# shanice-l/UNOPose

Measured on AMD Instinct MI355X. Metric: (query,ref) pairs/sec forward, higher is better.
Workload: dtype bf16; 1 GPU; UNOPose.forward, batch 32 pairs/GPU, 2048 query pts, 5000->2048 reference pts, 196 coarse pts, 518x518 crops, DINOv2 ViT-B/14 reg4, random-init (trained-like) weights

## Files before the change

unopose_amd/csrc/attn.hip:

```cpp
#include "gemm_common.h"

namespace unopose {

template <int XOR>
__device__ __forceinline__ float swz_xor(float v) {
  constexpr int ctrl = XOR == 1 ? 0xB1 : XOR == 2 ? 0x4E : XOR == 4 ? 0x141 : 0x140;
  return __int_as_float(__builtin_amdgcn_update_dpp(0, __float_as_int(v), ctrl, 0xF, 0xF, false));
}
__device__ __forceinline__ float row16_max(float v) {
  v = fmaxf(v, swz_xor<1>(v));
  v = fmaxf(v, swz_xor<2>(v));
  v = fmaxf(v, swz_xor<4>(v));
  v = fmaxf(v, swz_xor<8>(v));
  return v;
}
__device__ __forceinline__ float row16_sum(float v) {
  v += swz_xor<1>(v);
  v += swz_xor<2>(v);
  v += swz_xor<4>(v);
  v += swz_xor<8>(v);
  return v;
}

__device__ __forceinline__ bf16x8 zero8() {
  bf16x8 z;
#pragma unroll
  for (int i = 0; i < 8; ++i) z[i] = (__bf16)0.f;
  return z;
}

constexpr int TA_NT = 14;
constexpr int TA_MP = TA_NT * 16;

template <bool RPE, int RW>
__global__ __launch_bounds__(256, 2) void token_attn_kernel(const u16 *__restrict__ q, int ldq,
                                                         const u16 *__restrict__ k, int ldk,
                                                         const u16 *__restrict__ vt, const u16 *__restrict__ qp,
                                                         int ldqp, const u16 *__restrict__ E, int n, int m,
                                                         float scale, u16 *__restrict__ out) {
  __shared__ __attribute__((aligned(16))) u16 Pl[4][16][TA_MP];
  __shared__ __attribute__((aligned(16))) u16 Al[RPE ? 4 : 1][8][64][8];
  const int b = blockIdx.y, lane = threadIdx.x & 63, wave = threadIdx.x >> 6;
  const int n0 = (blockIdx.x * 4 + wave) * RW;
  if (n0 >= n) return;
  const int li = lane & 15, kg = lane >> 4;
  const int a_nl = li >> 2, a_h = li & 3;
  const bool a_valid = a_nl < RW && n0 + a_nl < n;
  const u16 *Q = q + ((size_t)b * n + n0 + a_nl) * ldq;
  const u16 *K = k + (size_t)b * m * ldk;

  f32x4 acc[TA_NT];
#pragma unroll
  for (int t = 0; t < TA_NT; ++t) acc[t] = f32x4{0.f, 0.f, 0.f, 0.f};

  {
    bf16x8 qa[8];
#pragma unroll
    for (int ks = 0; ks < 8; ++ks) {
      const int kk = ks * 32 + kg * 8;
      qa[ks] = zero8();
      if (a_valid && (kk >> 6) == a_h) qa[ks] = *reinterpret_cast<const bf16x8 *>(Q + kk);
    }
    bf16x8 kb[2][TA_NT];
    auto load_k = [&](int ks, bf16x8 (&dst)[TA_NT]) {
#pragma unroll
      for (int t = 0; t < TA_NT; ++t) {
        const int mm = min(t * 16 + li, m - 1);
        dst[t] = *reinterpret_cast<const bf16x8 *>(K + (size_t)mm * ldk + ks * 32 + kg * 8);
      }
    };
    load_k(0, kb[0]);
#pragma unroll
    for (int ks = 0; ks < 8; ++ks) {
      if (ks + 1 < 8) load_k(ks + 1, kb[(ks + 1) & 1]);
#pragma unroll
      for (int t = 0; t < TA_NT; ++t) acc[t] = __builtin_amdgcn_mfma_f32_16x16x32_bf16(qa[ks], kb[ks & 1][t], acc[t], 0, 0, 0);
    }
  }
  if (RPE) {
    for (int nl = 0; nl < RW; ++nl) {
      if (n0 + nl >= n) break;
      const u16 *QP = qp + ((size_t)b * n + n0 + nl) * ldqp + a_h * 256;
      const u16 *En = E + ((size_t)b * n + n0 + nl) * (size_t)m * 256;
#pragma unroll
      for (int ks = 0; ks < 8; ++ks) {
        bf16x8 av = zero8();
        if (a_nl == nl) av = *reinterpret_cast<const bf16x8 *>(QP + ks * 32 + kg * 8);
        *reinterpret_cast<bf16x8 *>(&Al[wave][ks][lane][0]) = av;
      }
      const int nt_valid = (m + 15) >> 4;
      bf16x8 buf[3][8];
      auto load_tile = [&](int t, bf16x8 (&dst)[8]) {
        const u16 *Er = En + (size_t)min(t * 16 + li, m - 1) * 256 + kg * 8;
#pragma unroll
        for (int ks = 0; ks < 8; ++ks) dst[ks] = *reinterpret_cast<const bf16x8 *>(Er + ks * 32);
      };
      load_tile(0, buf[0]);
      if (1 < nt_valid) load_tile(1, buf[1]);
#pragma unroll
      for (int t = 0; t < TA_NT; ++t) {
        if (t >= nt_valid) continue;
        if (t + 2 < nt_valid) load_tile(t + 2, buf[(t + 2) % 3]);
#pragma unroll
        for (int ks = 0; ks < 8; ++ks) {
          const bf16x8 av = *reinterpret_cast<const bf16x8 *>(&Al[wave][ks][lane][0]);
          acc[t] = __builtin_amdgcn_mfma_f32_16x16x32_bf16(av, buf[t % 3][ks], acc[t], 0, 0, 0);
        }
      }
    }
  }
  float mx[4] = {-3e38f, -3e38f, -3e38f, -3e38f};
#pragma unroll
  for (int t = 0; t < TA_NT; ++t) {
    const bool ok = t * 16 + li < m;
#pragma unroll
    for (int h = 0; h < 4; ++h) {
      acc[t][h] = ok ? acc[t][h] * scale : -3e38f;
      mx[h] = fmaxf(mx[h], acc[t][h]);
    }
  }
  float sm[4];
#pragma unroll
  for (int h = 0; h < 4; ++h) {
    mx[h] = row16_max(mx[h]);
    sm[h] = 0.f;
  }
#pragma unroll
  for (int t = 0; t < TA_NT; ++t) {
    const bool ok = t * 16 + li < m;
#pragma unroll
    for (int h = 0; h < 4; ++h) {
      const float p = ok ? __expf(acc[t][h] - mx[h]) : 0.f;
      acc[t][h] = p;
      sm[h] += p;
    }
  }
#pragma unroll
  for (int h = 0; h < 4; ++h) sm[h] = 1.f / row16_sum(sm[h]);
#pragma unroll
  for (int t = 0; t < TA_NT; ++t)
#pragma unroll
    for (int h = 0; h < 4; ++h) Pl[wave][kg * 4 + h][t * 16 + li] = f2bf(acc[t][h] * sm[h]);
  __builtin_amdgcn_fence(__ATOMIC_RELEASE, "wavefront");
  __builtin_amdgcn_wave_barrier();
  __builtin_amdgcn_fence(__ATOMIC_ACQUIRE, "wavefront");
  bf16x8 pa[TA_MP / 32];
#pragma unroll
  for (int ks = 0; ks < TA_MP / 32; ++ks)
    pa[ks] = *reinterpret_cast<const bf16x8 *>(&Pl[wave][li][ks * 32 + kg * 8]);
  const u16 *VT = vt + (size_t)b * 256 * TA_MP;
  constexpr int PK = TA_MP / 32;
  bf16x8 vb[2][PK];
  auto load_v = [&](int nt, bf16x8 (&dst)[PK]) {
    const u16 *Vr = VT + (size_t)(nt * 16 + li) * TA_MP + kg * 8;
#pragma unroll
    for (int ks = 0; ks < PK; ++ks) dst[ks] = *reinterpret_cast<const bf16x8 *>(Vr + ks * 32);
  };
  load_v(0, vb[0]);
#pragma unroll
  for (int nt = 0; nt < 16; ++nt) {
    if (nt + 1 < 16) load_v(nt + 1, vb[(nt + 1) & 1]);
    f32x4 o = f32x4{0.f, 0.f, 0.f, 0.f};
#pragma unroll
    for (int ks = 0; ks < PK; ++ks) o = __builtin_amdgcn_mfma_f32_16x16x32_bf16(pa[ks], vb[nt & 1][ks], o, 0, 0, 0);
    if (kg < RW && n0 + kg < n) out[((size_t)b * n + n0 + kg) * 256 + nt * 16 + li] = f2bf(o[nt >> 2]);
  }
}

constexpr int TA_EPOL = 1;
constexpr int TA_RING = 2 * 8192;
constexpr int TA_ROWS = 4;

__global__ __launch_bounds__(256, 2) void token_attn_rpe_dma_kernel(const u16 *__restrict__ q, int ldq, const u16 *__restrict__ k, int ldk,
                                                                     const u16 *__restrict__ vt, const u16 *__restrict__ qp, int ldqp,
                                                                     const u16 *__restrict__ E, int n, int m, float scale, int B,
                                                                     u16 *__restrict__ out) {
  constexpr int RW = 4;
  __shared__ __attribute__((aligned(1024))) char ring[4][TA_RING];
  const int b = blockIdx.y, lane = threadIdx.x & 63, wave = __builtin_amdgcn_readfirstlane(threadIdx.x >> 6);
  const int li = lane & 15, kg = lane >> 4;
  const int a_nl = li >> 2, a_h = li & 3;
  const int nbase = (blockIdx.x * 4 + wave) * TA_ROWS;
#pragma unroll 1
  for (int n0 = nbase; n0 < min(n, nbase + TA_ROWS); n0 += RW) {
  const int rw_here = min(RW, min(n, nbase + TA_ROWS) - n0);
  const bool a_valid = a_nl < rw_here;
  const u16 *Q = q + ((size_t)b * n + n0 + a_nl) * ldq;
  const u16 *K = k + (size_t)b * m * ldk;

  f32x4 acc[TA_NT];
#pragma unroll
  for (int t = 0; t < TA_NT; ++t) acc[t] = f32x4{0.f, 0.f, 0.f, 0.f};
  const uint32_t lds0 = (uint32_t)(uintptr_t)(__attribute__((address_space(3))) char *)&ring[0][0] + (uint32_t)wave * TA_RING;
  const int nt_valid = (m + 15) >> 4;
  const int rows_w = rw_here;
  const int total = rows_w * nt_valid;
  const __amdgpu_buffer_rsrc_t e_rs = __builtin_amdgcn_make_buffer_rsrc((void *)E, 0, (int)min((size_t)B * n * m * 512, (size_t)0xFFFFFFFFu), 0x00020000);
  uint32_t voff[8];
#pragma unroll
  for (int j = 0; j < 8; ++j) {
    const int key = 2 * j + (lane >> 5);
    voff[j] = (uint32_t)(key * 512 + (((lane & 31) ^ key) << 4));
  }
  const uint32_t row0 = (uint32_t)(((size_t)b * n + n0) * (size_t)m * 512);
  auto issue_tile = [&](int s) {
    const int r = s / nt_valid, t = s - r * nt_valid;
    const uint32_t so = row0 + (uint32_t)r * (uint32_t)m * 512u + (uint32_t)t * 8192u;
    const uint32_t dst = lds0 + (uint32_t)(s & 1) * 8192u;
#pragma unroll
    for (int j = 0; j < 8; ++j) gemm_dma16<TA_EPOL>(dst + j * 1024, so + voff[j], e_rs, 0);
  };
  issue_tile(0);
  if (total > 1) issue_tile(1);
  bf16x8 myq[8];
  {
    const u16 *QP = qp + ((size_t)b * n + n0 + a_nl) * ldqp + a_h * 256;
#pragma unroll
    for (int ks = 0; ks < 8; ++ks) {
      myq[ks] = zero8();
      if (a_valid) myq[ks] = *reinterpret_cast<const bf16x8 *>(QP + ks * 32 + kg * 8);
    }
  }
  {
    bf16x8 qa[8];
#pragma unroll
    for (int ks = 0; ks < 8; ++ks) {
      const int kk = ks * 32 + kg * 8;
      qa[ks] = zero8();
      if (a_valid && (kk >> 6) == a_h) qa[ks] = *reinterpret_cast<const bf16x8 *>(Q + kk);
    }
    bf16x8 kb[2][TA_NT];
    auto load_k = [&](int ks, bf16x8 (&dst)[TA_NT]) {
#pragma unroll
      for (int t = 0; t < TA_NT; ++t) {
        const int mm = min(t * 16 + li, m - 1);
        dst[t] = *reinterpret_cast<const bf16x8 *>(K + (size_t)mm * ldk + ks * 32 + kg * 8);
      }
    };
    load_k(0, kb[0]);
#pragma unroll
    for (int ks = 0; ks < 8; ++ks) {
      if (ks + 1 < 8) load_k(ks + 1, kb[(ks + 1) & 1]);
#pragma unroll
      for (int t = 0; t < TA_NT; ++t) acc[t] = __builtin_amdgcn_mfma_f32_16x16x32_bf16(qa[ks], kb[ks & 1][t], acc[t], 0, 0, 0);
    }
  }
  const char *ringw = &ring[0][0] + wave * TA_RING;
  const uint32_t frag_off = (uint32_t)(li * 512);
  int s = 0;
  for (int nl = 0; nl < rows_w; ++nl) {
    bf16x8 av[8];
#pragma unroll
    for (int ks = 0; ks < 8; ++ks) av[ks] = a_nl == nl ? myq[ks] : zero8();
#pragma unroll
    for (int t = 0; t < TA_NT; ++t) {
      if (t >= nt_valid) continue;
      if (s + 1 < total)
        asm volatile("s_waitcnt vmcnt(8)" ::: "memory");
      else
        asm volatile("s_waitcnt vmcnt(0)" ::: "memory");
      __builtin_amdgcn_sched_barrier(0);
      const char *tb = ringw + (s & 1) * 8192;
      bf16x8 eb[8];
#pragma unroll
      for (int ks = 0; ks < 8; ++ks) eb[ks] = *reinterpret_cast<const bf16x8 *>(tb + frag_off + ((((ks << 2) | kg) ^ li) << 4));
      asm volatile("s_waitcnt lgkmcnt(0)" ::: "memory");
      __builtin_amdgcn_sched_barrier(0);
      if (s + 2 < total) issue_tile(s + 2);
#pragma unroll
      for (int ks = 0; ks < 8; ++ks) acc[t] = __builtin_amdgcn_mfma_f32_16x16x32_bf16(av[ks], eb[ks], acc[t], 0, 0, 0);
      ++s;
    }
  }
  float mx[4] = {-3e38f, -3e38f, -3e38f, -3e38f};
#pragma unroll
  for (int t = 0; t < TA_NT; ++t) {
    const bool ok = t * 16 + li < m;
#pragma unroll
    for (int h = 0; h < 4; ++h) {
      acc[t][h] = ok ? acc[t][h] * scale : -3e38f;
      mx[h] = fmaxf(mx[h], acc[t][h]);
    }
  }
  float sm[4];
#pragma unroll
  for (int h = 0; h < 4; ++h) {
    mx[h] = row16_max(mx[h]);
    sm[h] = 0.f;
  }
#pragma unroll
  for (int t = 0; t < TA_NT; ++t) {
    const bool ok = t * 16 + li < m;
#pragma unroll
    for (int h = 0; h < 4; ++h) {
      const float p = ok ? __expf(acc[t][h] - mx[h]) : 0.f;
      acc[t][h] = p;
      sm[h] += p;
    }
  }
#pragma unroll
  for (int h = 0; h < 4; ++h) sm[h] = 1.f / row16_sum(sm[h]);
  u16(*Pl)[TA_MP] = reinterpret_cast<u16(*)[TA_MP]>(const_cast<char *>(ringw));
#pragma unroll
  for (int t = 0; t < TA_NT; ++t)
#pragma unroll
    for (int h = 0; h < 4; ++h) Pl[kg * 4 + h][t * 16 + li] = f2bf(acc[t][h] * sm[h]);
  __builtin_amdgcn_fence(__ATOMIC_RELEASE, "wavefront");
  __builtin_amdgcn_wave_barrier();
  __builtin_amdgcn_fence(__ATOMIC_ACQUIRE, "wavefront");
  bf16x8 pa[TA_MP / 32];
#pragma unroll
  for (int ks = 0; ks < TA_MP / 32; ++ks) pa[ks] = *reinterpret_cast<const bf16x8 *>(&Pl[li][ks * 32 + kg * 8]);
  const u16 *VT = vt + (size_t)b * 256 * TA_MP;
  constexpr int PK = TA_MP / 32;
  bf16x8 vb[2][PK];
  auto load_v = [&](int nt, bf16x8 (&dst)[PK]) {
    const u16 *Vr = VT + (size_t)(nt * 16 + li) * TA_MP + kg * 8;
#pragma unroll
    for (int ks = 0; ks < PK; ++ks) dst[ks] = *reinterpret_cast<const bf16x8 *>(Vr + ks * 32);
  };
  load_v(0, vb[0]);
#pragma unroll
  for (int nt = 0; nt < 16; ++nt) {
    if (nt + 1 < 16) load_v(nt + 1, vb[(nt + 1) & 1]);
    f32x4 o = f32x4{0.f, 0.f, 0.f, 0.f};
#pragma unroll
    for (int ks = 0; ks < PK; ++ks) o = __builtin_amdgcn_mfma_f32_16x16x32_bf16(pa[ks], vb[nt & 1][ks], o, 0, 0, 0);
    if (kg < rw_here) out[((size_t)b * n + n0 + kg) * 256 + nt * 16 + li] = f2bf(o[nt >> 2]);
  }
  asm volatile("s_waitcnt lgkmcnt(0)" ::: "memory");
  }
}

}

using namespace unopose;

extern "C" {

int unopose_token_attention(const void *q, int ldq, const void *k, int ldk, const void *vt, const void *qp, int ldqp,
                            const void *E, int B, int n, int m, float scale, void *out, unopose_stream_t stream) {
  UNOPOSE_REQUIRE(q && k && vt && out, "token_attention: null pointer");
  UNOPOSE_REQUIRE((qp == nullptr) == (E == nullptr), "token_attention: qp and E go together");
  UNOPOSE_REQUIRE(B >= 0 && n >= 1 && m >= 1 && m <= TA_MP && B <= 65535,
                  "token_attention: m=%d exceeds the %d-key tile", m, TA_MP);
  UNOPOSE_REQUIRE(ldq >= 256 && ldk >= 256 && ldq % 8 == 0 && ldk % 8 == 0 && (!E || (ldqp >= 1024 && ldqp % 8 == 0)),
                  "token_attention: row strides must be multiples of 8 elements (16-byte loads)");
  if (B == 0) return UNOPOSE_OK;
  hipStream_t s = (hipStream_t)stream;
  const bool dma = E && (size_t)B * n * m * 512 < (1UL << 32);
  if (dma) {
    static bool opt[64];
    if (lds_optin(opt, (const void *)token_attn_rpe_dma_kernel, 4 * TA_RING, "token_attention") != UNOPOSE_OK) return UNOPOSE_ELAUNCH;
    hipLaunchKernelGGL(token_attn_rpe_dma_kernel, dim3(cdiv(n, 4 * TA_ROWS), B), dim3(256), 0, s, (const u16 *)q, ldq, (const u16 *)k, ldk, (const u16 *)vt,
                       (const u16 *)qp, ldqp, (const u16 *)E, n, m, scale, B, (u16 *)out);
  } else if (E)
    hipLaunchKernelGGL((token_attn_kernel<true, 4>), dim3(cdiv(n, 16), B), dim3(256), 0, s, (const u16 *)q,
                       ldq, (const u16 *)k, ldk, (const u16 *)vt, (const u16 *)qp, ldqp, (const u16 *)E, n, m, scale,
                       (u16 *)out);
  else
    hipLaunchKernelGGL((token_attn_kernel<false, 4>), dim3(cdiv(n, 16), B), dim3(256), 0, s, (const u16 *)q,
                       ldq, (const u16 *)k, ldk, (const u16 *)vt, (const u16 *)nullptr, 0, (const u16 *)nullptr, n, m,
                       scale, (u16 *)out);
  return check_launch("token_attention");
}

int unopose_token_attention_key_pad(void) { return TA_MP; }

}
```

Before: 1138 pairs/s.

## Split RPE DMA ring into three half-tile slots with piece-counted waits

The per-wave LDS ring for streaming the relative-position embedding tiles moves from two 8 KiB tiles to three 4 KiB half-tiles. Each 16-key MMA step now reads its two halves from consecutive slots and issues refills one slot at a time, with vmcnt waits derived from a count of issued pieces. Per-workgroup LDS drops from 64 KiB to 48 KiB, which could allow more workgroups per CU and removes the opt-in call, while keeping roughly three slots of loads in flight. The cost is more complex wait and issue bookkeeping, runtime switches on the wait count, and partial-tile edge handling that could be wrong for odd m.

```diff
diff --git a/unopose_amd/csrc/attn.hip b/unopose_amd/csrc/attn.hip
--- a/unopose_amd/csrc/attn.hip
+++ b/unopose_amd/csrc/attn.hip
@@ -168,8 +168,21 @@
 }
 
 constexpr int TA_EPOL = 1;
-constexpr int TA_RING = 2 * 8192;
+constexpr int TA_SLOT = 4096;
+constexpr int TA_SLOTS = 3;
+constexpr int TA_RING = TA_SLOTS * TA_SLOT;
 constexpr int TA_ROWS = 4;
+
+static_assert((TA_SLOTS - 1) * 4 <= 8, "ta_wait_pieces: add cases");
+__device__ __forceinline__ void ta_wait_pieces(int left) {
+#define TA_WAIT_CASE(K) \
+  case K: asm volatile("s_waitcnt vmcnt(" #K ")" ::: "memory"); break;
+  switch (__builtin_amdgcn_readfirstlane(left)) {
+    TA_WAIT_CASE(0) TA_WAIT_CASE(1) TA_WAIT_CASE(2) TA_WAIT_CASE(3) TA_WAIT_CASE(4) TA_WAIT_CASE(5) TA_WAIT_CASE(6) TA_WAIT_CASE(7)
+    default: asm volatile("s_waitcnt vmcnt(8)" ::: "memory"); break;
+  }
+#undef TA_WAIT_CASE
+}
 
 __global__ __launch_bounds__(256, 2) void token_attn_rpe_dma_kernel(const u16 *__restrict__ q, int ldq, const u16 *__restrict__ k, int ldk,
                                                                      const u16 *__restrict__ vt, const u16 *__restrict__ qp, int ldqp,
@@ -194,24 +207,43 @@
   const uint32_t lds0 = (uint32_t)(uintptr_t)(__attribute__((address_space(3))) char *)&ring[0][0] + (uint32_t)wave * TA_RING;
   const int nt_valid = (m + 15) >> 4;
   const int rows_w = rw_here;
-  const int total = rows_w * nt_valid;
+  const int ns = (m + 7) >> 3;
+  const int row_pieces = (m + 1) >> 1;
+  const int total = rows_w * ns;
   const __amdgpu_buffer_rsrc_t e_rs = __builtin_amdgcn_make_buffer_rsrc((void *)E, 0, (int)min((size_t)B * n * m * 512, (size_t)0xFFFFFFFFu), 0x00020000);
-  uint32_t voff[8];
-#pragma unroll
-  for (int j = 0; j < 8; ++j) {
+  uint32_t voff[4];
+#pragma unroll
+  for (int j = 0; j < 4; ++j) {
     const int key = 2 * j + (lane >> 5);
     voff[j] = (uint32_t)(key * 512 + (((lane & 31) ^ key) << 4));
   }
   const uint32_t row0 = (uint32_t)(((size_t)b * n + n0) * (size_t)m * 512);
-  auto issue_tile = [&](int s) {
-    const int r = s / nt_valid, t = s - r * nt_valid;
-    const uint32_t so = row0 + (uint32_t)r * (uint32_t)m * 512u + (uint32_t)t * 8192u;
-    const uint32_t dst = lds0 + (uint32_t)(s & 1) * 8192u;
-#pragma unroll
-    for (int j = 0; j < 8; ++j) gemm_dma16<TA_EPOL>(dst + j * 1024, so + voff[j], e_rs, 0);
+  int i_slot = 0, i_ring = 0, issued = 0, p_issued = 0;
+  uint32_t i_row = row0;
+  auto issue_slot = [&]() {
+    const int np = min(4, row_pieces - 4 * i_slot);
+    const uint32_t flip = (uint32_t)(i_slot & 1) << 7;
+    const uint32_t so = i_row + (uint32_t)i_slot * 4096u;
+    const uint32_t dst = lds0 + (uint32_t)i_ring * TA_SLOT;
+    if (np == 4) {
+#pragma unroll
+      for (int j = 0; j < 4; ++j) gemm_dma16<TA_EPOL>(dst + j * 1024, so + (voff[j] ^ flip), e_rs, 0);
+    } else {
+      gemm_dma16<TA_EPOL>(dst, so + (voff[0] ^ flip), e_rs, 0);
+      if (np > 1) gemm_dma16<TA_EPOL>(dst + 1024, so + (voff[1] ^ flip), e_rs, 0);
+      if (np > 2) gemm_dma16<TA_EPOL>(dst + 2048, so + (voff[2] ^ flip), e_rs, 0);
+    }
+    p_issued += np;
+    ++issued;
+    i_ring = i_ring == TA_SLOTS - 1 ? 0 : i_ring + 1;
+    if (++i_slot == ns) {
+      i_slot = 0;
+      i_row += (uint32_t)m * 512u;
+    }
   };
-  issue_tile(0);
-  if (total > 1) issue_tile(1);
+#pragma unroll
+  for (int u = 0; u < TA_SLOTS; ++u)
+    if (issued < total) issue_slot();
   bf16x8 myq[8];
   {
     const u16 *QP = qp + ((size_t)b * n + n0 + a_nl) * ldqp + a_h * 256;
@@ -246,8 +278,8 @@
     }
   }
   const char *ringw = &ring[0][0] + wave * TA_RING;
-  const uint32_t frag_off = (uint32_t)(li * 512);
-  int s = 0;
+  const uint32_t frag_off = (uint32_t)((li & 7) * 512);
+  int c_ring = 0, p_need = 0;
   for (int nl = 0; nl < rows_w; ++nl) {
     bf16x8 av[8];
 #pragma unroll
@@ -255,21 +287,22 @@
 #pragma unroll
     for (int t = 0; t < TA_NT; ++t) {
       if (t >= nt_valid) continue;
-      if (s + 1 < total)
-        asm volatile("s_waitcnt vmcnt(8)" ::: "memory");
-      else
-        asm volatile("s_waitcnt vmcnt(0)" ::: "memory");
+      const int nslot = min(2, ns - 2 * t);
+      p_need += min(8, row_pieces - 8 * t);
+      ta_wait_pieces(p_issued - p_need);
       __builtin_amdgcn_sched_barrier(0);
-      const char *tb = ringw + (s & 1) * 8192;
+      const int c_next = c_ring == TA_SLOTS - 1 ? 0 : c_ring + 1;
+      const char *tb = ringw + ((li >> 3) ? c_next : c_ring) * TA_SLOT;
       bf16x8 eb[8];
 #pragma unroll
       for (int ks = 0; ks < 8; ++ks) eb[ks] = *reinterpret_cast<const bf16x8 *>(tb + frag_off + ((((ks << 2) | kg) ^ li) << 4));
       asm volatile("s_waitcnt lgkmcnt(0)" ::: "memory");
       __builtin_amdgcn_sched_barrier(0);
-      if (s + 2 < total) issue_tile(s + 2);
+      if (issued < total) issue_slot();
+      if (nslot == 2 && issued < total) issue_slot();
+      c_ring = nslot == 2 ? (c_next == TA_SLOTS - 1 ? 0 : c_next + 1) : c_next;
 #pragma unroll
       for (int ks = 0; ks < 8; ++ks) acc[t] = __builtin_amdgcn_mfma_f32_16x16x32_bf16(av[ks], eb[ks], acc[t], 0, 0, 0);
-      ++s;
     }
   }
   float mx[4] = {-3e38f, -3e38f, -3e38f, -3e38f};
@@ -350,8 +383,7 @@
   hipStream_t s = (hipStream_t)stream;
   const bool dma = E && (size_t)B * n * m * 512 < (1UL << 32);
   if (dma) {
-    static bool opt[64];
-    if (lds_optin(opt, (const void *)token_attn_rpe_dma_kernel, 4 * TA_RING, "token_attention") != UNOPOSE_OK) return UNOPOSE_ELAUNCH;
+    static_assert(4 * TA_RING <= 64 * 1024, "token_attention: a ring above 64 KiB per workgroup needs lds_optin");
     hipLaunchKernelGGL(token_attn_rpe_dma_kernel, dim3(cdiv(n, 4 * TA_ROWS), B), dim3(256), 0, s, (const u16 *)q, ldq, (const u16 *)k, ldk, (const u16 *)vt,
                        (const u16 *)qp, ldqp, (const u16 *)E, n, m, scale, B, (u16 *)out);
   } else if (E)
```

Result: no change. 1136 pairs/s (-0.1%).
